# supersglzc/pql

Hardware: AMD Instinct MI355X
Metric: learner grad-steps/sec + env-steps/sec, 4096 envs batch 8192 (value = V-learner grad-steps/s at the design schedule 1 env-iteration : 4 P-steps : 8 V-steps -- critic_sample_ratio 8, critic_actor_ratio 2; weak scaling: batch-sized steps summed over ranks, strong scaling: steps of the job's batch) (higher is better)
Workload: dtype f32; 1 GPU; PQL 1xMI355X: 4096 synthetic envs (AllegroHand-shape obs=88 act=16), replay 1000000 rows resident in HBM, batch 8192, n-step 3, DoubleQ MLP [512, 512, 256]; schedule=1 env-iteration : 4 P-steps : 8 V-steps, graph=True, rng=philox, streams=True, fused_forward=True, parallelism=single, layout=single, ranks=1

## Files before the change

### pql_amd/csrc/fused.h

```cpp
#pragma once
#include "pqlk_common.h"

typedef float f32x16f __attribute__((ext_vector_type(16)));

struct FusedP {
  const float* X;
  const float* X2;
  int ldx2, x2_col0;
  const float* params;
  const float* packed;
  float* acts;
  int B, ldx, n_hidden, stash_all, buf_ld, n_nets;
  int dims[PQLK_MAX_LAYERS + 1];
  long long net_stride, packed_net_stride;
  long long b_off[PQLK_MAX_LAYERS], p_off[PQLK_MAX_LAYERS], a_off[PQLK_MAX_LAYERS];
  int head_n, head_epi, head_ld, ld_out2;
  long long head_w_off, head_b_off, head_a_off;
  const float* draw;
  float* out2;
  float* qc;
  float noise_std, noise_clip;
  const float* td_qt;
  const float* td_rew;
  const float* td_done;
// ... 16 lines not shown

template <int R, int TPW, int TM, int D, bool REFILL>
__device__ __forceinline__ void fused_group(f32x16f (&acc)[R][TPW], float4 (&bq)[D][TM], const float4* const (&wp)[TPW],
                                            const float4* __restrict__ lds4, int abase, int buf_ld4, int k8, int K8, int steps,
                                            float4 (&an)[R]) {
#pragma unroll
  for (int s = 0; s < D; ++s) {
    if (s < steps) {
      float4 a[R];
      const int kq = min(k8 + s + 1, K8 - 1);
#pragma unroll
      for (int i = 0; i < R; ++i) { a[i] = an[i]; an[i] = lds4[abase + 32 * i * buf_ld4 + 2 * kq]; }
      __builtin_amdgcn_sched_barrier(0);
      const int kn = min(k8 + s + D, K8 - 1);
#pragma unroll
      for (int t = 0; t < 4; ++t) {
#pragma unroll
        for (int j = 0; j < TPW; ++j) {
          const float bv = t == 0 ? bq[s][j].x : t == 1 ? bq[s][j].y : t == 2 ? bq[s][j].z : bq[s][j].w;
#pragma unroll
          for (int i = 0; i < R; ++i) {
            const float av = t == 0 ? a[i].x : t == 1 ? a[i].y : t == 2 ? a[i].z : a[i].w;
            acc[i][j] = __builtin_amdgcn_mfma_f32_32x32x2f32(bv, av, acc[i][j], 0, 0, 0);
          }
          if (REFILL && t == 3) {
            bq[s][j] = wp[j][kn * 64];
            __builtin_amdgcn_sched_barrier(0);
          }
        }
      }
    }
  }
}

template <int TM, int D>
__device__ __forceinline__ void fused_ring_fill(float4 (&bq)[D][TM], const float4* __restrict__ packed_l, int K8, int K8s, int ntiles, int tpw,
                                                int wave, int lane) {
  const float4* w[TM];
#pragma unroll
  for (int j = 0; j < TM; ++j) w[j] = packed_l + (long long)min(wave * tpw + j, ntiles - 1) * K8s * 64 + lane;
#pragma unroll
  for (int s = 0; s < D; ++s) {
    const int ks = min(s, K8 - 1) * 64;
#pragma unroll
    for (int j = 0; j < TM; ++j) bq[s][j] = w[j][ks];
  }
}

template <int R, int TPW, int TM, int D>
__device__ __forceinline__ void fused_layer(float4 (&bq)[D][TM], int buf_ld4, int K8, int K8s, int ntiles, const float4* __restrict__ packed_l,
                                            int bias_lds4, float* __restrict__ gout, int g_ld, int row0, int B, int wave, int lane,
                                            const float4* __restrict__ packed_n, int K8n, int ntiles_n, int tpw_n,
                                            float* __restrict__ gprev, int nprev4) {
  const int r = lane & 31, h = lane >> 5;
  const int t0 = wave * TPW;
  const bool active = t0 < ntiles;
  const float4* lds4 = reinterpret_cast<const float4*>(fsm);
  float4* gprev4 = reinterpret_cast<float4*>(gprev) + (long long)row0 * nprev4;
  const int srows = gprev ? 32 * R : 0;
  const int tid = wave * 64 + lane;
  int srow = tid / nprev4, sc4 = tid % nprev4;
  const int sdq = (64 * FUSED_NW) / nprev4, sdm = (64 * FUSED_NW) % nprev4;
  f32x16f acc[R][TPW];
#pragma unroll
  for (int i = 0; i < R; ++i)
#pragma unroll
    for (int j = 0; j < TPW; ++j)
#pragma unroll
      for (int e = 0; e < 16; ++e) acc[i][j][e] = 0.f;
  if (active) {
    const float4* wp[TPW];
#pragma unroll
    for (int j = 0; j < TPW; ++j) wp[j] = packed_l + (long long)min(t0 + j, ntiles - 1) * K8s * 64 + lane;
    const int abase = r * buf_ld4 + h;
    const int K8full = K8 - (K8 % D);
    const int G = K8full / D;
    const bool rem = K8full < K8;
    float4 an[R];
#pragma unroll
    for (int i = 0; i < R; ++i) an[i] = lds4[abase + 32 * i * buf_ld4];
    if (G > 1) fused_group<R, TPW, TM, D, true>(acc, bq, wp, lds4, abase, buf_ld4, 0, K8, D, an);
    for (int g = 1; g < G - 1; ++g) {
      if (srow < srows) {
        gprev4[(long long)srow * nprev4 + sc4] = lds4[srow * buf_ld4 + sc4];
        srow += sdq; sc4 += sdm;
        if (sc4 >= nprev4) { sc4 -= nprev4; ++srow; }
      }
      fused_group<R, TPW, TM, D, true>(acc, bq, wp, lds4, abase, buf_ld4, g * D, K8, D, an);
    }
    if (G >= 1) {
      if (rem) fused_group<R, TPW, TM, D, true>(acc, bq, wp, lds4, abase, buf_ld4, (G - 1) * D, K8, D, an);
      else fused_group<R, TPW, TM, D, false>(acc, bq, wp, lds4, abase, buf_ld4, (G - 1) * D, K8, D, an);
    }
    if (rem) fused_group<R, TPW, TM, D, false>(acc, bq, wp, lds4, abase, buf_ld4, K8full, K8, K8 - K8full, an);
  }
  while (srow < srows) {
    gprev4[(long long)srow * nprev4 + sc4] = lds4[srow * buf_ld4 + sc4];
    srow += sdq; sc4 += sdm;
    if (sc4 >= nprev4) { sc4 -= nprev4; ++srow; }
  }
  if (packed_n) fused_ring_fill<TM, D>(bq, packed_n, K8n, K8n, ntiles_n, tpw_n, wave, lane);
  __syncthreads();
  if (active) {
    float4* out4 = reinterpret_cast<float4*>(fsm);
    const bool full = row0 + 32 * R <= B;
#pragma unroll
    for (int j = 0; j < TPW; ++j) {
      if (t0 + j < ntiles) {
#pragma unroll
        for (int q = 0; q < 4; ++q) {
          const int c4 = 8 * (t0 + j) + 2 * q + h;
          const float4 b4 = lds4[bias_lds4 + c4];
#pragma unroll
          for (int i = 0; i < R; ++i) {
            const int row = row0 + 32 * i + r;
            float4 v;
            v.x = fused_elu(acc[i][j][4 * q] + b4.x);
            v.y = fused_elu(acc[i][j][4 * q + 1] + b4.y);
            v.z = fused_elu(acc[i][j][4 * q + 2] + b4.z);
            v.w = fused_elu(acc[i][j][4 * q + 3] + b4.w);
            out4[(32 * i + r) * buf_ld4 + c4] = v;
            if (gout && (full || row < B)) *reinterpret_cast<float4*>(gout + (long long)row * g_ld + 4 * c4) = v;
          }
        }
      }
    }
  }
  __syncthreads();
}

enum { HEAD_NONE = PQLK_ACT_NONE, HEAD_TANH = PQLK_ACT_TANH, HEAD_TANH_NOISE = PQLK_ACT_TANH_NOISE };

template <int R, bool TDH = true>
__device__ __forceinline__ void fused_head(const FusedP& p, const float* __restrict__ params, float* __restrict__ acts, int net, int row0,
                                           int buf_ld4, int wave, int lane) {
  constexpr int NW = FUSED_NW;
  const int r = lane & 31, h = lane >> 5;
  const int Kh = p.dims[p.n_hidden], K8 = Kh >> 3, N = p.head_n;
  const float* W = params + (long long)net * p.net_stride + p.head_w_off;
  const float4* wp = reinterpret_cast<const float4*>(W + (long long)min(r, N - 1) * Kh) + h;
  const float4* lds4 = reinterpret_cast<const float4*>(fsm);
  const int per = (K8 + NW - 1) / NW, k0 = wave * per, k1 = min(K8, k0 + per);
  f32x16f acc[R];
#pragma unroll
  for (int i = 0; i < R; ++i)
#pragma unroll
    for (int e = 0; e < 16; ++e) acc[i][e] = 0.f;
  for (int k8 = k0; k8 < k1; ++k8) {
    const float4 w4 = wp[2 * k8];
#pragma unroll
    for (int i = 0; i < R; ++i) {
      const float4 a4 = lds4[(32 * i + r) * buf_ld4 + 2 * k8 + h];
      acc[i] = __builtin_amdgcn_mfma_f32_32x32x2f32(w4.x, a4.x, acc[i], 0, 0, 0);
      acc[i] = __builtin_amdgcn_mfma_f32_32x32x2f32(w4.y, a4.y, acc[i], 0, 0, 0);
      acc[i] = __builtin_amdgcn_mfma_f32_32x32x2f32(w4.z, a4.z, acc[i], 0, 0, 0);
      acc[i] = __builtin_amdgcn_mfma_f32_32x32x2f32(w4.w, a4.w, acc[i], 0, 0, 0);
    }
  }
  const bool td = TDH && p.td_dz != nullptr;
  constexpr int TDI = 2 * R;
  float tdt[TDI], tdr[TDI], tdd[TDI];
  if (td && ((wave * 64 + lane) & 31) == 0) {
#pragma unroll
    for (int k = 0; k < TDI; ++k) {
      const long long m = min(row0 + ((wave * 64 + lane) >> 5) + 16 * k, p.B - 1);
      tdt[k] = fminf(p.td_qt[m * p.head_ld], p.td_qt[((long long)p.B + m) * p.head_ld]);
      tdr[k] = p.td_rew[m]; tdd[k] = p.td_done[m];
    }
  }
  auto part_at = [&](int x) { return td ? (x >> 8) * p.buf_ld + Kh + (x & 255) : x; };
  __syncthreads();
#pragma unroll
  for (int i = 0; i < R; ++i)
#pragma unroll
    for (int e = 0; e < 16; ++e) fsm[part_at(((wave * R + i) * 16 + e) * 64 + lane)] = acc[i][e];
  __syncthreads();
  const float* bias = params + (long long)net * p.net_stride + p.head_b_off;
  float* out = acts + p.head_a_off + (long long)net * p.B * p.head_ld;
  const int tdbase = 32 * R * p.buf_ld;
  int ok = 0;
  for (int o = wave * 64 + lane; o < 32 * R * p.head_ld; o += 64 * NW, ++ok) {
    const int row = o / p.head_ld, c = o - row * p.head_ld;
    if (row0 + row >= p.B) {
      if (td && c == 0) { fsm[tdbase + row] = 0.f; fsm[tdbase + 32 * R + row] = 0.f; }
      continue;
    }
    float x = 0.f;
    if (c < N) {
      const int i = row >> 5, ln = (row & 31) + 32 * ((c >> 2) & 1), e = 4 * (c >> 3) + (c & 3);
      float s = 0.f;
#pragma unroll
      for (int w = 0; w < NW; ++w) s += fsm[part_at(((w * R + i) * 16 + e) * 64 + ln)];
      x = s + bias[c];
      if (p.qc) p.qc[(long long)net * p.B + row0 + row] = x;
      if (td) {
        float tq = tdt[0], tr = tdr[0], tn = tdd[0];
#pragma unroll
        for (int k = 1; k < TDI; ++k)
          if (ok == k) { tq = tdt[k]; tr = tdr[k]; tn = tdd[k]; }
        const float y = tr + ((1.f - tn) * p.td_gamma_n) * tq;
        const float dq = x - y;
        fsm[tdbase + row] = p.td_two_over_b * dq;
        fsm[tdbase + 32 * R + row] = dq * dq;
      }
      if (p.head_epi == HEAD_TANH) x = tanhf(x);
      else if (p.head_epi == HEAD_TANH_NOISE) {
        x = tanhf(x);
        float nz = p.noise_std * p.draw[(long long)(row0 + row) * N + c];
        nz = fminf(fmaxf(nz, -p.noise_clip), p.noise_clip);
        x = fminf(fmaxf(x + nz, -1.f), 1.f);
      }
      if (p.out2 && net == 0) p.out2[(long long)(row0 + row) * p.ld_out2 + c] = x;
    }
    out[(long long)(row0 + row) * p.head_ld + c] = x;
  }
  if (!td) return;
  __syncthreads();
  const int kq = Kh >> 2;
  const int tile = row0 / (32 * R);
  float* dz = p.td_dz + ((long long)net * p.B + row0) * Kh;
  constexpr int RW = 32 * R / NW;
  float* hp = p.td_head_part + ((long long)tile * p.n_nets + net) * p.td_part_floats;
  for (int q0 = 0; q0 < kq; q0 += 64) {
    const int q = q0 + lane;
    float4 s = make_float4(0.f, 0.f, 0.f, 0.f);
    if (q < kq) {
      const float4 w4 = *reinterpret_cast<const float4*>(W + 4 * q);
#pragma unroll
      for (int u = 0; u < RW; ++u) {
        const int row = wave * RW + u;
        const float dn = fsm[tdbase + row];
        const float4 h4 = lds4[row * buf_ld4 + q];
        s.x += dn * h4.x; s.y += dn * h4.y; s.z += dn * h4.z; s.w += dn * h4.w;
        float4 a = make_float4(dn * w4.x, dn * w4.y, dn * w4.z, dn * w4.w);
        a.x = h4.x > 0.f ? a.x : a.x * (h4.x + 1.f);
        a.y = h4.y > 0.f ? a.y : a.y * (h4.y + 1.f);
        a.z = h4.z > 0.f ? a.z : a.z * (h4.z + 1.f);
        a.w = h4.w > 0.f ? a.w : a.w * (h4.w + 1.f);
        if (row0 + row < p.B) *reinterpret_cast<float4*>(dz + (long long)row * Kh + 4 * q) = a;
      }
    }
    __syncthreads();
    if (q < kq) *reinterpret_cast<float4*>(&fsm[wave * p.buf_ld + Kh + 4 * lane]) = s;
    __syncthreads();
    if (wave == 0 && q < kq) {
      float4 t = *reinterpret_cast<const float4*>(&fsm[Kh + 4 * lane]);
#pragma unroll
      for (int w = 1; w < NW; ++w) {
        const float4 v = *reinterpret_cast<const float4*>(&fsm[w * p.buf_ld + Kh + 4 * lane]);
        t.x += v.x; t.y += v.y; t.z += v.z; t.w += v.w;
      }
      *reinterpret_cast<float4*>(hp + 4 * q) = t;
    }
  }
  if (wave == 1) {
    float db = lane < 32 * R ? fsm[tdbase + lane] : 0.f, ls = lane < 32 * R ? fsm[tdbase + 32 * R + lane] : 0.f;
    db = wave_sum(db); ls = wave_sum(ls);
    if (lane < 32) hp[Kh + lane] = lane == 0 ? db : 0.f;
    if (lane == 0) p.td_loss_part[(long long)tile * p.n_nets + net] = ls;
  }
}

template <int R, int TM, bool OUT_ONLY = false>
__global__ __launch_bounds__(64 * FUSED_NW) void k_mlp_fwd_fused(FusedP p) {
  constexpr int NW = FUSED_NW, D = TM >= 4 ? 2 : PQLK_FUSED_DEEP;
  const int tid = threadIdx.x, lane = tid & 63, wave = tid >> 6;
  int net, tile;
  const int tiles = (p.B + 32 * R - 1) / (32 * R);
  if (p.n_nets == 2 && (tiles & 3) == 0) {
    const int b = blockIdx.x, g = b & 7, i = b >> 3;
    net = g & 1;
    tile = i * 4 + (g >> 1);
  } else {
    net = blockIdx.x / tiles;
    tile = blockIdx.x % tiles;
  }
  const float* __restrict__ pX = p.X;
  const float* __restrict__ pparams = p.params;
  const float* __restrict__ ppacked = p.packed;
  float* __restrict__ pacts = p.acts;
  const int pstash = OUT_ONLY ? 0 : p.stash_all;
  const int row0 = tile * 32 * R;
  const bool full_tile = row0 + 32 * R <= p.B;
  const int buf_ld4 = p.buf_ld >> 2;
  const float4* packed_net = reinterpret_cast<const float4*>(ppacked + (long long)net * p.packed_net_stride);
  auto tpw_of = [](int ntiles) { return ntiles > 2 * NW ? 4 : ntiles > NW ? 2 : 1; };
  float4 bq[D][TM];
  fused_ring_fill<TM, D>(bq, packed_net + (p.p_off[0] >> 2), (p.dims[0] + 7) >> 3, ((p.dims[0] + 31) & ~31) >> 3, p.dims[1] >> 5,
                         tpw_of(p.dims[1] >> 5), wave, lane);
  float4* out4 = reinterpret_cast<float4*>(fsm);
  const int bias4 = 32 * R * buf_ld4;
  {
    float4 bv[PQLK_MAX_LAYERS];
#pragma unroll
    for (int l = 0; l < PQLK_MAX_LAYERS; ++l) {
      bv[l] = make_float4(0.f, 0.f, 0.f, 0.f);
      if (l < p.n_hidden && tid < (p.dims[l + 1] >> 2))
        bv[l] = reinterpret_cast<const float4*>(pparams + (long long)net * p.net_stride + p.b_off[l])[tid];
    }
    const int k0 = (p.dims[0] + 31) & ~31, cpr = k0 >> 2, w = p.dims[0], total = 32 * R * cpr;
    for (int i0 = tid; i0 < total; i0 += 4 * 64 * NW) {
      float4 v[4];
#pragma unroll
      for (int u = 0; u < 4; ++u) {
        const int i = i0 + u * 64 * NW;
        const int row = i / cpr, c4 = i - row * cpr;
        v[u] = make_float4(0.f, 0.f, 0.f, 0.f);
        if (i < total && row0 + row < p.B) {
          const int c = 4 * c4;
          if (p.X2 && c >= p.x2_col0) {
            if (c - p.x2_col0 < p.ldx2) v[u] = *reinterpret_cast<const float4*>(p.X2 + (long long)(row0 + row) * p.ldx2 + (c - p.x2_col0));
          } else if (c < p.ldx) {
            v[u] = *reinterpret_cast<const float4*>(pX + (long long)(row0 + row) * p.ldx + c);
          }
        }
      }
#pragma unroll
      for (int u = 0; u < 4; ++u) {
        const int i = i0 + u * 64 * NW;
        if (i < total) {
          const int row = i / cpr, c4 = i - row * cpr, c = 4 * c4;
          float4 x = v[u];
// ... 65 lines not shown
```

### pql_amd/csrc/gemm.hip

```cpp
#include <cstdlib>
#include <type_traits>
#include "pqlk_common.h"
#include "skinny.h"
#include "fused.h"

typedef float f32x16 __attribute__((ext_vector_type(16)));

enum { MODE_FWD = 0, MODE_DX = 1, MODE_DW = 2 };
enum { EPI_NONE = 0, EPI_ELU = 1, EPI_TANH = 2, EPI_TANH_NOISE = 3, EPI_DELU = 4, EPI_DTANH_SLICE = 5 };

struct GemmP {
  const float* A;
  const float* B;
  float* C;
  const float* bias;
  const float* aux;
  float* C2;
  float* dbias;
  int M, N, K;
  int lda, ldb, ldc, ldaux, ldc2;
  int ncols_store;
  long long sA, sB, sC, sBias, sAux;
  int groups;
  int zsum;
// ... 362 lines not shown
        __builtin_amdgcn_sched_barrier(0);
        compute(kt, 0);
        PQLK_SS(1, 1);
        __syncthreads();
        PQLK_GL(min(kt + 3, nk - 1), 1);
        __builtin_amdgcn_sched_barrier(0);
        compute(kt + 1, 1);
        PQLK_SS(0, 0);
        __syncthreads();
      }
#undef PQLK_GL
#undef PQLK_SS
      continue;
    }

    KcTile<BM, KT> a_kc;
    RrTile<BM, KT> a_rr;
    KcTile<BN, KT> b_kc;
    RrTile<BN, KT> b_rr;

    auto gload = [&](int kt) {
      const int k0 = kbeg + kt * KT;
      if (MODE == MODE_FWD) {
        a_kc.load(A, p.lda, m0, p.M, k0, kend, tid);
        b_kc.load(B, p.ldb, n0, p.N, k0, kend, tid);
      } else if (MODE == MODE_DX) {
        a_kc.load(A, p.lda, m0, p.M, k0, p.lda, tid);
        b_rr.load(B, p.ldb, k0, kend, n0, p.ldb, tid);
      } else {
        a_rr.load(A, p.lda, k0, kend, m0, p.lda, tid);
        b_rr.load(B, p.ldb, k0, kend, n0, p.ldb, tid);
      }
    };
    auto sstore = [&](int stage) {
      float* sa = smem + stage * S::STAGE;
      float* sb = sa + S::A_FLOATS;
      if (MODE == MODE_FWD) {
        a_kc.store(sa, tid);
        b_kc.store(sb, tid);
      } else if (MODE == MODE_DX) {
        a_kc.store(sa, tid);
        b_rr.store(sb, tid);
      } else {
        a_rr.store(sa, tid);
        b_rr.store(sb, tid);
      }
    };

    gload(0);
    __syncthreads();
    sstore(0);
    __syncthreads();

    for (int kt = 0; kt < nk; ++kt) {
      const int stage = kt & 1;
      if (kt + 1 < nk) gload(kt + 1);
      compute(kt, stage);
      if (kt + 1 < nk) sstore(stage ^ 1);
      __syncthreads();
    }
  }

  if (MODE == MODE_DW && bx == 0) {
    smem[tid] = dbacc;
    __syncthreads();
    if (tid < BM) {
      dbacc = smem[tid];
#pragma unroll
      for (int g = 1; g < 256 / BM; ++g) dbacc += smem[g * BM + tid];
    }
    __syncthreads();
  }
  if (MODE != MODE_FWD && EPI != EPI_DTANH_SLICE) {
    const bool whole = (m0 + BM <= p.M) && (n0 + BN <= p.N) && (MODE == MODE_DW || !p.C2);
    if (whole) {
      constexpr int PLD = WN + 4;
      constexpr int LPR = WN / 4;
      constexpr int RPI = 64 / LPR;
      float* patch = smem + wave * (32 * PLD);
      const int gq = (MODE == MODE_DX && p.zsum) ? 0 : g0;
      float* Cw = (MODE == MODE_DW) ? p.C + (long long)g0 * p.sC + (long long)split * p.sSplit : p.C + (long long)gq * p.sC;
      const float* auxw = (EPI == EPI_DELU && p.aux) ? p.aux + (long long)gq * p.sAux : nullptr;
      const int prow = lane / LPR, pc4 = lane % LPR;
#pragma unroll
      for (int i = 0; i < MI; ++i) {
        f4v h4s[(EPI == EPI_DELU) ? 32 / RPI : 1];
        if (EPI == EPI_DELU) {
          long long arow[32 / RPI];
          const long long grow0 = m0 + wm + 32 * i + prow;
          if (MODE == MODE_DX && p.perm) {
            int pr[32 / RPI];
#pragma unroll
            for (int it = 0; it < 32 / RPI; ++it) pr[it] = p.perm[grow0 + it * RPI];
#pragma unroll
            for (int it = 0; it < 32 / RPI; ++it) arow[it] = pr[it] < 0 ? 0 : pr[it];
          } else {
#pragma unroll
            for (int it = 0; it < 32 / RPI; ++it) arow[it] = grow0 + it * RPI;
          }
#pragma unroll
          for (int it = 0; it < 32 / RPI; ++it)
            h4s[it] = *reinterpret_cast<const f4v*>(auxw + arow[it] * p.ldaux + n0 + wn + 4 * pc4);
        }
#pragma unroll
        for (int j = 0; j < NJ; ++j)
#pragma unroll
          for (int q = 0; q < 4; ++q)
            *reinterpret_cast<float4*>(patch + r * PLD + 32 * j + 8 * q + 4 * h) =
                make_float4(acc[i][j][4 * q], acc[i][j][4 * q + 1], acc[i][j][4 * q + 2], acc[i][j][4 * q + 3]);
        __builtin_amdgcn_fence(__ATOMIC_RELEASE, "wavefront");
        __builtin_amdgcn_wave_barrier();
        __builtin_amdgcn_fence(__ATOMIC_ACQUIRE, "wavefront");
#pragma unroll
        for (int it = 0; it < 32 / RPI; ++it) {
          const int rr = it * RPI + prow;
          float4 v = *reinterpret_cast<const float4*>(patch + rr * PLD + 4 * pc4);
          const long long grow = m0 + wm + 32 * i + rr;
          const int gcol = n0 + wn + 4 * pc4;
          if (EPI == EPI_DELU) {
            const f4v h4 = h4s[it];
            v.x = h4.x > 0.f ? v.x : v.x * (h4.x + 1.f);
            v.y = h4.y > 0.f ? v.y : v.y * (h4.y + 1.f);
            v.z = h4.z > 0.f ? v.z : v.z * (h4.z + 1.f);
            v.w = h4.w > 0.f ? v.w : v.w * (h4.w + 1.f);
          }
          *reinterpret_cast<float4*>(Cw + grow * p.ldc + gcol) = v;
        }
        if (i + 1 < MI) {
          __builtin_amdgcn_fence(__ATOMIC_RELEASE, "wavefront");
          __builtin_amdgcn_wave_barrier();
          __builtin_amdgcn_fence(__ATOMIC_ACQUIRE, "wavefront");
        }
      }
      if (MODE == MODE_DW && bx == 0 && tid < BM && p.dbias) {
        float* db = p.dbias + (long long)g0 * p.sBias + (long long)split * p.sSplit;
        const int row = m0 + tid;
        if (row < p.ncols_store) db[row] = row < p.M ? dbacc : 0.f;
      }
      return;
    }
  }
  if (MODE == MODE_DW) {
    float* C = p.C + (long long)g0 * p.sC + (long long)split * p.sSplit;
#pragma unroll
    for (int i = 0; i < MI; ++i)
#pragma unroll
      for (int j = 0; j < NJ; ++j) {
        const int row = m0 + wm + 32 * i + r;
#pragma unroll
        for (int q = 0; q < 4; ++q) {
          const int col = n0 + wn + 32 * j + 8 * q + 4 * h;
          if (row < p.M && col < p.N)
            *reinterpret_cast<float4*>(C + (long long)row * p.ldc + col) =
                make_float4(acc[i][j][4 * q], acc[i][j][4 * q + 1], acc[i][j][4 * q + 2], acc[i][j][4 * q + 3]);
        }
      }
    if (bx == 0 && tid < BM && p.dbias) {
      float* db = p.dbias + (long long)g0 * p.sBias + (long long)split * p.sSplit;
      const int row = m0 + tid;
      if (row < p.ncols_store) db[row] = row < p.M ? dbacc : 0.f;
    }
    return;
  }

  const int g = (MODE == MODE_DX && p.zsum) ? 0 : g0;
  float* C = p.C + (long long)g * p.sC;
  const float* bias = (MODE == MODE_FWD && p.bias) ? p.bias + (long long)g * p.sBias : nullptr;
  const float* aux = p.aux ? p.aux + (long long)g * p.sAux : nullptr;
  const bool full = (m0 + BM <= p.M) && (n0 + BN <= p.N) && EPI != EPI_DTANH_SLICE && EPI != EPI_TANH_NOISE && !p.C2;
#pragma unroll
  for (int i = 0; i < MI; ++i)
#pragma unroll
    for (int j = 0; j < NJ; ++j) {
      const int row = m0 + wm + 32 * i + r;
#pragma unroll
      for (int q = 0; q < 4; ++q) {
        const int col = n0 + wn + 32 * j + 8 * q + 4 * h;
        float v[4] = {acc[i][j][4 * q], acc[i][j][4 * q + 1], acc[i][j][4 * q + 2], acc[i][j][4 * q + 3]};
        if (full) {
          if (MODE == MODE_FWD) {
            const float4 b4 = bias ? *reinterpret_cast<const float4*>(bias + col) : make_float4(0.f, 0.f, 0.f, 0.f);
            v[0] += b4.x; v[1] += b4.y; v[2] += b4.z; v[3] += b4.w;
#pragma unroll
            for (int u = 0; u < 4; ++u) {
              if (EPI == EPI_ELU) v[u] = elu1(v[u]);
              else if (EPI == EPI_TANH) v[u] = tanhf(v[u]);
            }
          } else if (EPI == EPI_DELU) {
            const float4 h4 = *reinterpret_cast<const float4*>(aux + (long long)row * p.ldaux + col);
            v[0] = h4.x > 0.f ? v[0] : v[0] * (h4.x + 1.f);
            v[1] = h4.y > 0.f ? v[1] : v[1] * (h4.y + 1.f);
            v[2] = h4.z > 0.f ? v[2] : v[2] * (h4.z + 1.f);
            v[3] = h4.w > 0.f ? v[3] : v[3] * (h4.w + 1.f);
          }
          *reinterpret_cast<float4*>(C + (long long)row * p.ldc + col) = make_float4(v[0], v[1], v[2], v[3]);
          continue;
        }
        if (row >= p.M) continue;
#pragma unroll
        for (int u = 0; u < 4; ++u) {
          const int c = col + u;
          float x = v[u];
          if (EPI == EPI_DTANH_SLICE) {
            const int cc = c - p.col0;
            if (cc >= 0 && cc < p.ncol) {
              const float a = aux[(long long)row * p.ldaux + cc];
              C[(long long)row * p.ldc + cc] = x * (1.f - a * a);
            }
            continue;
// ... 358 lines not shown
  int rc = desc_ok(d);
  if (rc) return rc;
  PQLK_REQUIRE(params && x && acts, PQLK_E_NULL);
  PQLK_REQUIRE(b > 0 && b < (1LL << 30), PQLK_E_SHAPE);
  PQLK_REQUIRE(ldx % 32 == 0 && ldx >= pqlk_ld(d->dims[0]), PQLK_E_ALIGN);
  PQLK_REQUIRE(pqlk_aligned16(params) && pqlk_aligned16(x) && pqlk_aligned16(acts), PQLK_E_ALIGN);
  PQLK_REQUIRE(out_act == PQLK_ACT_NONE || out_act == PQLK_ACT_TANH || out_act == PQLK_ACT_TANH_NOISE, PQLK_E_UNSUPPORTED);
  if (out_act == PQLK_ACT_TANH_NOISE) PQLK_REQUIRE(draw, PQLK_E_NULL);
  if (out2) PQLK_REQUIRE(d->n_nets == 1 && ld_out2 >= d->dims[d->n_layers], PQLK_E_SHAPE);
  PQLK_REQUIRE(stash_all >= 0 && stash_all <= PQLK_STASH_OUTPUT_ONLY, PQLK_E_RANGE);
  const int64_t net_stride = pqlk_mlp_net_stride(d);
  const int L = d->n_layers;
  int l_first = 0;
  static const bool no_head = getenv("PQLK_NO_FUSED_HEAD") != nullptr;
  const bool out_only = stash_all == PQLK_STASH_OUTPUT_ONLY;
  if (out_only) PQLK_REQUIRE(packed && fusable(d, nullptr) && head_fusable(d) && !no_head, PQLK_E_UNSUPPORTED);
  if (packed && fusable(d, nullptr)) {
    PQLK_REQUIRE(pqlk_aligned16(packed), PQLK_E_ALIGN);
    FusedHead head = {};
    if (head_fusable(d) && !no_head) {
      head.n = d->dims[L]; head.epi = out_act; head.draw = draw; head.noise_std = noise_std; head.noise_clip = noise_clip;
      head.out2 = out2; head.ld_out2 = ld_out2;
    }
    rc = launch_fused_hidden(d, params, packed, x, ldx, b, acts, stash_all == 1 ? 1 : 0, pqlk_s(stream), &head, out_only);
    if (rc) return rc;
    l_first = head.n > 0 ? L : L - 1;
  }
  for (int l = l_first; l < L; ++l) {
    int64_t w_off, b_off, a_off, a_ld;
    pqlk_mlp_layer_offsets(d, l, &w_off, &b_off);
    pqlk_mlp_act_offset(d, b, 0, l, &a_off, &a_ld);
    GemmP p = {};
    if (l == 0) {
      p.A = x; p.lda = (int)ldx; p.sA = 0;
    } else {
      int64_t i_off, i_ld;
      pqlk_mlp_act_offset(d, b, 0, l - 1, &i_off, &i_ld);
      p.A = acts + i_off; p.lda = (int)i_ld; p.sA = b * i_ld;
    }
    p.B = params + w_off; p.ldb = (int)pqlk_ld(d->dims[l]); p.sB = net_stride;
    p.bias = params + b_off; p.sBias = net_stride;
    p.C = acts + a_off; p.ldc = (int)a_ld; p.sC = b * a_ld;
    p.M = (int)b; p.N = d->dims[l + 1]; p.K = (int)pqlk_ld(d->dims[l]);
    p.ncols_store = (int)a_ld;
    p.groups = d->n_nets;
    p.epi = EPI_ELU;
    if (l == L - 1) {
      p.epi = out_act == PQLK_ACT_TANH ? EPI_TANH : (out_act == PQLK_ACT_TANH_NOISE ? EPI_TANH_NOISE : EPI_NONE);
      p.aux = draw; p.sAux = 0;
      p.noise_std = noise_std; p.noise_clip = noise_clip;
      p.C2 = out2; p.ldc2 = (int)ld_out2;
    }
    if (l == L - 1 && skinny_fwd_ok(d->dims[l + 1], p.K)) {
      SkinnyP q = {};
      q.X = p.A; q.ldx = p.lda; q.sX = p.sA;
      q.W = p.B; q.ldk = p.ldb; q.sW = p.sB;
      q.bias = p.bias; q.sBias = p.sBias;
      q.C = p.C; q.ldc = p.ldc; q.sC = p.sC;
      q.M = p.M; q.N = p.N; q.K = p.K;
      q.epi = p.epi == EPI_TANH ? SK_EPI_TANH : (p.epi == EPI_TANH_NOISE ? SK_EPI_TANH_NOISE : SK_EPI_NONE);
      q.draw = p.aux; q.noise_std = noise_std; q.noise_clip = noise_clip;
      q.C2 = p.C2; q.ldc2 = p.ldc2;
      rc = launch_skinny_fwd(q, d->n_nets, pqlk_s(stream));
    } else if (l == L - 1 && narrow_fwd_ok(p)) {
      rc = launch_fwd_narrow(p, d->n_nets, pqlk_s(stream));
    } else {
      rc = launch_auto<MODE_FWD>(p, d->n_nets, pqlk_s(stream));
    }
    if (rc) return rc;
  }
  return PQLK_OK;
}

struct ReduceP {
  const float* slabs; int splits; long long n;
  float* out;
  const float* head_part; int head_parts; int n_nets; long long net_stride, head_off, head_floats;
  long long seg_off, seg_len;
  int main_blocks;
  float* sq_part; int32_t* step_dev;
  const int* parts_dev;
};

__global__ __launch_bounds__(256) void k_reduce_slabs(ReduceP p) {
  __shared__ float shw[4];
  float acc = 0.f;
  if ((int)blockIdx.x < p.main_blocks) {
    const long long sq = p.seg_len >> 2, n4 = sq * p.n_nets;
    for (long long i = (long long)blockIdx.x * 256 + threadIdx.x; i < n4; i += (long long)p.main_blocks * 256) {
      long long q = i, base = p.seg_off;
      while (q >= sq) { q -= sq; base += p.net_stride; }
      if (p.head_parts > 0 && p.seg_off + (q << 2) >= p.head_off) continue;
      const long long off = base + (q << 2);
      float4 s = *reinterpret_cast<const float4*>(p.slabs + off);
      for (int k = 1; k < p.splits; ++k) {
        const float4 t = *reinterpret_cast<const float4*>(p.slabs + (long long)k * p.n + off);
        s.x += t.x; s.y += t.y; s.z += t.z; s.w += t.w;
      }
      *reinterpret_cast<float4*>(p.out + off) = s;
      acc += (s.x * s.x + s.y * s.y) + (s.z * s.z + s.w * s.w);
    }
    if (!p.sq_part) return;
    acc = wave_sum(acc);
  } else {
    const int lane = threadIdx.x & 63;
    const long long hq = p.head_floats >> 2;
    const long long e = ((long long)blockIdx.x - p.main_blocks) * 4 + (threadIdx.x >> 6);
    if (e < hq * p.n_nets) {
      const long long net = e / hq, q = e - net * hq;
      const float* hp = p.head_part + net * p.head_floats + 4 * q;
      float4 s = make_float4(0.f, 0.f, 0.f, 0.f);
      const int parts = p.parts_dev ? min(p.head_parts, (p.parts_dev[3] + 31) / 32) : p.head_parts;
      for (int k = lane; k < parts; k += 64) {
        const float4 t = *reinterpret_cast<const float4*>(hp + (long long)k * p.n_nets * p.head_floats);
        s.x += t.x; s.y += t.y; s.z += t.z; s.w += t.w;
      }
      s.x = wave_sum(s.x); s.y = wave_sum(s.y); s.z = wave_sum(s.z); s.w = wave_sum(s.w);
      if (lane == 0) *reinterpret_cast<float4*>(p.out + net * p.net_stride + p.head_off + 4 * q) = s;
      acc = (s.x * s.x + s.y * s.y) + (s.z * s.z + s.w * s.w);
    }
    if (!p.sq_part) return;
  }
  if ((threadIdx.x & 63) == 0) shw[threadIdx.x >> 6] = acc;
  __syncthreads();
  if (threadIdx.x == 0) {
    p.sq_part[blockIdx.x] = (shw[0] + shw[1]) + (shw[2] + shw[3]);
    if (blockIdx.x == 0 && p.step_dev) p.step_dev[0] += 1;
  }
}

static int64_t head_quads(const PqlMlpDesc* d) {
  const int L = d->n_layers;
  return ((int64_t)d->dims[L] * pqlk_ld(d->dims[L - 1]) + pqlk_ld(d->dims[L])) / 4 * d->n_nets;
}
static bool head_is_fused(const PqlMlpDesc* d) {
  const int L = d->n_layers;
  return L >= 2 && skinny_bwd_ok(d->dims[L], (int)pqlk_ld(d->dims[L - 1])) && skinny_bwd_fused_ok(d->dims[L], (int)pqlk_ld(d->dims[L - 1]));
}
static int reduce_main_blocks(int64_t arena, bool for_norm) {
  int64_t blocks = (arena / 4 + 255) / 256;
  if (blocks < 1) blocks = 1;
  const int64_t cap = for_norm ? 1024 : 2048;
  return (int)(blocks > cap ? cap : blocks);
}

extern "C" int32_t pqlk_mlp_norm_parts(const PqlMlpDesc* d) {
  if (desc_ok(d)) return 0;
  const int main_blocks = reduce_main_blocks(pqlk_mlp_param_floats(d), true);
  return main_blocks + (head_is_fused(d) ? (int)((head_quads(d) + 3) / 4) : 0);
}

struct TdHead {
  const float* qt; const float* rew; const float* done; float gamma_n; float* loss_part;
};

static int mlp_backward_impl(const PqlMlpDesc* d, const float* params, const float* x, int64_t ldx, int64_t b,
                             const float* acts, const float* dy, float* grads, int32_t splits, float* dx,
                             int64_t ld_dx, int32_t dx_col0, int32_t dx_cols, const float* dx_tanh_of,
                             int64_t ld_tanh, float* ws, int64_t ws_floats, float* sq_part, int32_t* step_dev,
                             pqlk_stream_t stream, const TdHead* td = nullptr, int l_hi = -1, int l_lo = 0, int head_done = 0,
                             const int* head_parts_dev = nullptr) {
  int rc = desc_ok(d);
  if (rc) return rc;
  const bool ranged = l_hi >= 0;
  if (!ranged) l_hi = d->n_layers - 1;
  PQLK_REQUIRE(l_lo >= 0 && l_lo <= l_hi && l_hi < d->n_layers, PQLK_E_RANGE);
  PQLK_REQUIRE(!ranged || (grads && !dx && !sq_part), PQLK_E_UNSUPPORTED);
  PQLK_REQUIRE(params && x && acts && (dy || td || head_done || l_hi < d->n_layers - 1) && ws, PQLK_E_NULL);
  PQLK_REQUIRE(!head_done || (!ranged && grads && !dx && !td && d->n_layers >= 2), PQLK_E_UNSUPPORTED);
  if (td) PQLK_REQUIRE(grads && d->n_nets == 2 && d->dims[d->n_layers] == 1 && head_is_fused(d), PQLK_E_UNSUPPORTED);
  PQLK_REQUIRE(b > 0 && b < (1LL << 30), PQLK_E_SHAPE);
  PQLK_REQUIRE(ldx % 32 == 0 && ldx >= pqlk_ld(d->dims[0]), PQLK_E_ALIGN);
  PQLK_REQUIRE(grads || dx, PQLK_E_NULL);
  if (grads) PQLK_REQUIRE(splits >= 1 && splits <= 64, PQLK_E_SHAPE);
  if (!grads) splits = 0;
  PQLK_REQUIRE(ws_floats >= 2 * (int64_t)d->n_nets * b * max_hidden_ld(d) + (int64_t)splits * pqlk_mlp_param_floats(d) +
                                (grads ? head_part_floats(d, b) : 0), PQLK_E_WORKSPACE);
  PQLK_REQUIRE(!sq_part || grads, PQLK_E_NULL);
  if (dx) {
    PQLK_REQUIRE(ld_dx % 32 == 0, PQLK_E_ALIGN);
// ... 43 lines not shown
          pqlk_mlp_act_offset(d, b, 0, L - 1, &q_off, &q_ld);
          PQLK_REQUIRE(in_ld >= ld_in && q_ld == ld_out, PQLK_E_SHAPE);
          q.td_q = acts + q_off; q.td_qt = td->qt; q.td_rew = td->rew; q.td_done = td->done;
          q.td_gamma_n = td->gamma_n; q.td_two_over_b = 2.0f / (float)b; q.td_part = td->loss_part;
        }
        rc = launch_skinny_bwd(q, d->n_nets, head_part, (long long)(net_stride - w_off), st);
        if (rc) return rc;
        continue;
      }
      if (grads) {
        q.dW = slabs + w_off; q.dB = slabs + b_off; q.sW = net_stride; q.sBias = net_stride; q.sSplit = arena;
        q.splits = splits; q.rows_per_split = (int)pqlk_round_up((b + splits - 1) / splits, KT_MAX);
        rc = launch_skinny_dw(q, d->n_nets, st);
        if (rc) return rc;
      }
      if (l > 0) {
        q.W = params + w_off; q.sW = net_stride;
        q.C = dact[flip]; q.sC = b * ld_in;
        q.epi = SK_EPI_DELU;
        rc = launch_skinny_dx(q, d->n_nets, st);
        if (rc) return rc;
        continue;
      }
      if (!dx) continue;
    }
    if (grads && !skinny) {
      GemmP p = {};
      p.A = cur_dy; p.lda = (int)ld_out; p.sA = b * ld_out;
      p.B = in; p.ldb = (int)in_ld; p.sB = in_stride;
      p.C = slabs + w_off; p.ldc = (int)ld_in; p.sC = net_stride;
      p.dbias = slabs + b_off; p.sBias = net_stride;
      p.M = d->dims[l + 1]; p.N = (int)ld_in; p.K = (int)b;
      p.ncols_store = (int)ld_out;
      p.groups = d->n_nets; p.splits = splits;
      p.rows_per_split = (int)pqlk_round_up((b + splits - 1) / splits, KT_MAX);
      p.sSplit = arena;
      rc = launch_auto<MODE_DW>(p, d->n_nets * splits, st);
      if (rc) return rc;
    }
    if (l > 0) {
      GemmP p = {};
      p.A = cur_dy; p.lda = (int)ld_out; p.sA = b * ld_out;
      p.B = params + w_off; p.ldb = (int)ld_in; p.sB = net_stride;
      p.C = dact[flip]; p.ldc = (int)ld_in; p.sC = b * ld_in;
      p.aux = in; p.ldaux = (int)in_ld; p.sAux = in_stride;
      p.M = (int)b; p.N = d->dims[l]; p.K = d->dims[l + 1];
      p.ncols_store = (int)ld_in;
      p.groups = d->n_nets; p.zsum = 0;
      p.epi = EPI_DELU;
      rc = launch_auto<MODE_DX>(p, d->n_nets, st);
      if (rc) return rc;
    } else if (dx) {
      GemmP p = {};
      p.A = cur_dy; p.lda = (int)ld_out; p.sA = b * ld_out;
      p.B = params + w_off; p.ldb = (int)ld_in; p.sB = net_stride;
      p.C = dx; p.ldc = (int)ld_dx; p.sC = 0;
      p.M = (int)b; p.N = d->dims[0]; p.K = d->dims[1];
      p.ncols_store = (int)ld_in;
      p.groups = d->n_nets; p.zsum = 1;
      if (dx_tanh_of) {
        p.epi = EPI_DTANH_SLICE; p.aux = dx_tanh_of; p.ldaux = (int)ld_tanh; p.col0 = dx_col0; p.ncol = dx_cols;
      } else {
        p.epi = EPI_NONE;
      }
      if (dx_slice_ok(p)) rc = launch_dx_slice(p, st);
      else rc = launch_auto<MODE_DX>(p, 1, st);
      if (rc) return rc;
    }
  }
  if (grads) {
    ReduceP r = {};
    r.slabs = slabs; r.splits = splits; r.n = arena; r.out = grads;
    r.head_part = head_part; r.head_parts = head_blocks; r.n_nets = d->n_nets; r.net_stride = net_stride;
    int64_t w_last, b_last, w_lo, w_next, b_tmp;
    pqlk_mlp_layer_offsets(d, L - 1, &w_last, &b_last);
    r.head_off = w_last; r.head_floats = net_stride - w_last;
    pqlk_mlp_layer_offsets(d, l_lo, &w_lo, &b_tmp);
    w_next = net_stride;
    if (l_hi < L - 1) pqlk_mlp_layer_offsets(d, l_hi + 1, &w_next, &b_tmp);
    r.seg_off = w_lo; r.seg_len = w_next - w_lo;
    r.sq_part = sq_part; r.step_dev = step_dev; r.parts_dev = head_parts_dev;
    r.main_blocks = reduce_main_blocks(r.seg_len * d->n_nets, sq_part != nullptr);
    const int extra = head_blocks > 0 ? (int)((head_quads(d) + 3) / 4) : 0;
    hipLaunchKernelGGL(k_reduce_slabs, dim3(r.main_blocks + extra), dim3(256), 0, st, r);
    PQLK_LAUNCH_CHECK();
  }
  return PQLK_OK;
}

static bool minnet_ok(const PqlMlpDesc* d, const float* dx, const float* dx_tanh_of, int dx_cols) {
  const int L = d->n_layers;
  if (d->n_nets != 2 || L < 3 || d->dims[L] != 1 || !dx || !dx_tanh_of || dx_cols > 32) return false;
  if (!skinny_bwd_ok(1, (int)pqlk_ld(d->dims[L - 1]))) return false;
  for (int l = 1; l < L; ++l)
    if (d->dims[l] % 32 != 0) return false;
  for (int l = 1; l < L - 1; ++l)
    if (d->dims[l] % 128 != 0) return false;
  return true;
}
static int64_t minnet_rows_cap(int64_t b) { return 2 * pqlk_round_up(b, MN_TILE); }

static int launch_compact_dx(const GemmP& p, bool first, hipStream_t st) {
  static const int ctile = [] { const char* e = getenv("PQLK_COMPACT_TILE"); return e ? atoi(e) : 2; }();
  const bool small = ctile == 2 || (ctile == 3 && first) || (ctile == 4 && !first);
  if (ctile == 1) return launch_gemm<MODE_DX, 128, 128, EPI_DELU>(p, 1, st);
  if (small) return launch_gemm<MODE_DX, 64, 64, EPI_DELU>(p, 1, st);
  return launch_gemm<MODE_DX, 128, 64, EPI_DELU>(p, 1, st);
}

extern "C" int64_t pqlk_dpg_backward_ws_floats(const PqlMlpDesc* d, int64_t b) {
  if (desc_ok(d) || b <= 0) return 0;
  const int64_t dense = pqlk_mlp_bwd_ws_floats(d, b, 1);
  const int64_t compact = 2 * minnet_rows_cap(b) * max_hidden_ld(d) + 2 * minnet_rows_cap(b) + 64;
  return dense > compact ? dense : compact;
}

extern "C" int pqlk_dpg_critic_backward(const PqlMlpDesc* d, const float* params, const float* x, int64_t ldx, int64_t b,
                                        const float* acts, const float* dy, float* dx, int64_t ld_dx, int32_t dx_col0,
                                        int32_t dx_cols, const float* dx_tanh_of, int64_t ld_tanh, const uint8_t* owner, float* ws,
                                        int64_t ws_floats, pqlk_stream_t stream) {
  int rc = desc_ok(d);
  if (rc) return rc;
  PQLK_REQUIRE(ws_floats >= pqlk_dpg_backward_ws_floats(d, b), PQLK_E_WORKSPACE);
  if (!minnet_ok(d, dx, dx_tanh_of, dx_cols) || b > 131072)
    return mlp_backward_impl(d, params, x, ldx, b, acts, dy, nullptr, 1, dx, ld_dx, dx_col0, dx_cols, dx_tanh_of, ld_tanh, ws, ws_floats,
                             nullptr, nullptr, stream);
  PQLK_REQUIRE(params && acts && dy && ws, PQLK_E_NULL);
  PQLK_REQUIRE(b > 0 && b < (1LL << 29), PQLK_E_SHAPE);
  PQLK_REQUIRE(ld_dx % 32 == 0 && dx_col0 >= 0 && dx_cols > 0 && dx_col0 + dx_cols <= d->dims[0] && ld_dx >= dx_cols, PQLK_E_RANGE);
  const int L = d->n_layers;
  const int64_t net_stride = pqlk_mlp_net_stride(d);
  const int64_t rows_cap = minnet_rows_cap(b), mld = max_hidden_ld(d);
  float* dz[2] = {ws, ws + rows_cap * mld};
  int* perm = reinterpret_cast<int*>(ws + 2 * rows_cap * mld);
  int* mn = perm + rows_cap;
  hipStream_t st = pqlk_s(stream);
  int64_t q_off, q_ld;
  pqlk_mlp_act_offset(d, b, 0, L - 1, &q_off, &q_ld);
  hipLaunchKernelGGL(k_minnet_partition, dim3(1), dim3(1024), 0, st, owner, acts + q_off, q_ld, b, perm, rows_cap, mn);
  PQLK_LAUNCH_CHECK();
  {
    int64_t w_off, b_off, h_off, h_ld;
    pqlk_mlp_layer_offsets(d, L - 1, &w_off, &b_off);
    pqlk_mlp_act_offset(d, b, 0, L - 2, &h_off, &h_ld);
    MinnetHeadP h = {};
    h.H = acts + h_off; h.sH = b * h_ld; h.ldh = (int)h_ld;
    h.W = params + w_off; h.sW = net_stride; h.ldk = (int)pqlk_ld(d->dims[L - 1]);
    h.dY = dy; h.sY = b * pqlk_ld(1); h.ldy = (int)pqlk_ld(1);
    h.C = dz[0]; h.perm = perm; h.mn = mn; h.N = 1; h.K = h.ldk; h.rows_cap = rows_cap;
    h.zero_out = dx; h.zero_floats = b * ld_dx;
    int64_t blocks = rows_cap / 4;
    if (blocks > 2048) blocks = 2048;
    hipLaunchKernelGGL(k_minnet_head_dx, dim3((unsigned)blocks), dim3(256), (size_t)2 * h.N * h.K * sizeof(float), st, h);
    PQLK_LAUNCH_CHECK();
  }
  int flip = 0;
  for (int l = L - 2; l >= 1; --l) {
    int64_t w_off, b_off, a_off, a_ld;
    pqlk_mlp_layer_offsets(d, l, &w_off, &b_off);
    pqlk_mlp_act_offset(d, b, 0, l - 1, &a_off, &a_ld);
    GemmP p = {};
    p.A = dz[flip]; p.lda = (int)pqlk_ld(d->dims[l + 1]); p.sA = 0;
    p.B = params + w_off; p.ldb = (int)pqlk_ld(d->dims[l]); p.sB = net_stride;
    p.C = dz[flip ^ 1]; p.ldc = (int)pqlk_ld(d->dims[l]); p.sC = 0;
    p.aux = acts + a_off; p.ldaux = (int)a_ld; p.sAux = b * a_ld;
    p.M = (int)rows_cap; p.N = d->dims[l]; p.K = d->dims[l + 1];
    p.ncols_store = p.ldc;
// ... 294 lines not shown
```

### pql_amd/csrc/pqlk_common.h

```cpp
#pragma once
#include <hip/hip_runtime.h>
#include <stdint.h>

#include <atomic>
#include <mutex>

#include "../../include/pqlk.h"

#define PQLK_WAVE 64

#define PQLK_REQUIRE(cond, code) \
  do {                           \
    if (!(cond)) return (code);  \
  } while (0)

#define PQLK_LAUNCH_CHECK()                    \
  do {                                         \
    hipError_t e__ = hipGetLastError();        \
    if (e__ != hipSuccess) return -(int)e__;   \
  } while (0)

static inline int64_t pqlk_round_up(int64_t x, int64_t m) { return (x + m - 1) / m * m; }
static inline hipStream_t pqlk_s(pqlk_stream_t s) { return (hipStream_t)s; }
static inline bool pqlk_aligned16(const void* p) { return (((uintptr_t)p) & 15u) == 0; }

struct RecLayout {
  int O, A;
  int o4, a4;
  int off_nobs, off_act, off_rd;
  int used;
  int ld;
};

__host__ __device__ static inline RecLayout rec_layout(int O, int A) {
  RecLayout L;
  L.O = O; L.A = A;
  L.o4 = (O + 3) & ~3;
  if (A < 0) {
    L.a4 = 0; L.off_nobs = L.off_act = L.off_rd = L.o4; L.used = L.o4;
  } else {
    L.a4 = (A + 3) & ~3;
    L.off_nobs = L.o4; L.off_act = 2 * L.o4; L.off_rd = 2 * L.o4 + L.a4; L.used = L.off_rd + 4;
  }
  L.ld = (L.used + 31) & ~31;
  return L;
}

struct RecLayoutH {
  int O, A;
  int oh;
  int off_nobs, off_act, off_rd;
  int used;
  int ld;
};

__host__ __device__ static inline RecLayoutH rec_layout_h(int O, int A) {
  RecLayoutH L;
  L.O = O; L.A = A;
  L.oh = ((O + 7) & ~7) >> 1;
  if (A < 0) {
    L.off_nobs = L.off_act = L.off_rd = L.oh; L.used = L.oh;
  } else {
    L.off_nobs = L.oh; L.off_act = 2 * L.oh; L.off_rd = 2 * L.oh + ((A + 3) & ~3); L.used = L.off_rd + 4;
  }
  L.ld = (L.used + 31) & ~31;
  return L;
}

struct PqlkPerDeviceOnce {
  std::atomic<bool> done[64] = {};
  std::mutex mu;
  template <class F>
  int run(F&& f) {
    int dev = 0;
    if (hipGetDevice(&dev) != hipSuccess || dev < 0 || dev >= 64) return f();
    if (done[dev].load(std::memory_order_acquire)) return 0;
    std::lock_guard<std::mutex> g(mu);
    if (done[dev].load(std::memory_order_relaxed)) return 0;
    const int rc = f();
    if (rc == 0) done[dev].store(true, std::memory_order_release);
    return rc;
  }
};

__device__ __forceinline__ float wave_sum(float v) {
#pragma unroll
  for (int o = 32; o > 0; o >>= 1) v += __shfl_xor(v, o, 64);
  return v;
}
__device__ __forceinline__ float wave_max(float v) {
#pragma unroll
  for (int o = 32; o > 0; o >>= 1) v = fmaxf(v, __shfl_xor(v, o, 64));
  return v;
}
```

Baseline: 1218 V-learner grad-steps/s.

## Use write-through buffer stores for activations and templated split reduction

Adds a helper that issues raw buffer b128 stores with a cache-policy bit, and uses it for activation stash, dz, and backward GEMM epilogue stores. Full-tile activation writes to global memory move to a coalesced pass from LDS after the barrier. The slab reduction kernel gets compile-time split counts (8 and 16) so loads can be unrolled and issued together. The intent is to cut cache pollution and store overhead and to raise memory-level parallelism in the reduction. The cost is 32-bit offset limits in the buffer resource (int indices) and an extra LDS read pass.

```diff
diff --git a/pql_amd/csrc/fused.h b/pql_amd/csrc/fused.h
--- a/pql_amd/csrc/fused.h
+++ b/pql_amd/csrc/fused.h
@@ -122,7 +122,7 @@
     if (G > 1) fused_group<R, TPW, TM, D, true>(acc, bq, wp, lds4, abase, buf_ld4, 0, K8, D, an);
     for (int g = 1; g < G - 1; ++g) {
       if (srow < srows) {
-        gprev4[(long long)srow * nprev4 + sc4] = lds4[srow * buf_ld4 + sc4];
+        pqlk_store_wt(gprev4, srow * nprev4 + sc4, lds4[srow * buf_ld4 + sc4]);
         srow += sdq; sc4 += sdm;
         if (sc4 >= nprev4) { sc4 -= nprev4; ++srow; }
       }
@@ -135,7 +135,7 @@
     if (rem) fused_group<R, TPW, TM, D, false>(acc, bq, wp, lds4, abase, buf_ld4, K8full, K8, K8 - K8full, an);
   }
   while (srow < srows) {
-    gprev4[(long long)srow * nprev4 + sc4] = lds4[srow * buf_ld4 + sc4];
+    pqlk_store_wt(gprev4, srow * nprev4 + sc4, lds4[srow * buf_ld4 + sc4]);
     srow += sdq; sc4 += sdm;
     if (sc4 >= nprev4) { sc4 -= nprev4; ++srow; }
   }
@@ -160,13 +160,21 @@
             v.z = fused_elu(acc[i][j][4 * q + 2] + b4.z);
             v.w = fused_elu(acc[i][j][4 * q + 3] + b4.w);
             out4[(32 * i + r) * buf_ld4 + c4] = v;
-            if (gout && (full || row < B)) *reinterpret_cast<float4*>(gout + (long long)row * g_ld + 4 * c4) = v;
+            if (gout && !full && row < B) *reinterpret_cast<float4*>(gout + (long long)row * g_ld + 4 * c4) = v;
           }
         }
       }
     }
   }
   __syncthreads();
+  if (gout && row0 + 32 * R <= B) {
+    float4* g4 = reinterpret_cast<float4*>(gout + (long long)row0 * g_ld);
+    const int n4 = g_ld >> 2, total = 32 * R * n4;
+    for (int e = tid; e < total; e += 64 * FUSED_NW) {
+      const int row = e / n4;
+      pqlk_store_wt(g4, e, lds4[row * buf_ld4 + (e - row * n4)]);
+    }
+  }
 }
 
 enum { HEAD_NONE = PQLK_ACT_NONE, HEAD_TANH = PQLK_ACT_TANH, HEAD_TANH_NOISE = PQLK_ACT_TANH_NOISE };
@@ -277,7 +285,7 @@
         a.y = h4.y > 0.f ? a.y : a.y * (h4.y + 1.f);
         a.z = h4.z > 0.f ? a.z : a.z * (h4.z + 1.f);
         a.w = h4.w > 0.f ? a.w : a.w * (h4.w + 1.f);
-        if (row0 + row < p.B) *reinterpret_cast<float4*>(dz + (long long)row * Kh + 4 * q) = a;
+        if (row0 + row < p.B) pqlk_store_wt(reinterpret_cast<float4*>(dz), row * kq + q, a);
       }
     }
     __syncthreads();
diff --git a/pql_amd/csrc/gemm.hip b/pql_amd/csrc/gemm.hip
--- a/pql_amd/csrc/gemm.hip
+++ b/pql_amd/csrc/gemm.hip
@@ -468,6 +468,7 @@
       float* Cw = (MODE == MODE_DW) ? p.C + (long long)g0 * p.sC + (long long)split * p.sSplit : p.C + (long long)gq * p.sC;
       const float* auxw = (EPI == EPI_DELU && p.aux) ? p.aux + (long long)gq * p.sAux : nullptr;
       const int prow = lane / LPR, pc4 = lane % LPR;
+      float4* Cb = reinterpret_cast<float4*>(Cw + (long long)m0 * p.ldc + n0);
 #pragma unroll
       for (int i = 0; i < MI; ++i) {
         f4v h4s[(EPI == EPI_DELU) ? 32 / RPI : 1];
@@ -501,8 +502,6 @@
         for (int it = 0; it < 32 / RPI; ++it) {
           const int rr = it * RPI + prow;
           float4 v = *reinterpret_cast<const float4*>(patch + rr * PLD + 4 * pc4);
-          const long long grow = m0 + wm + 32 * i + rr;
-          const int gcol = n0 + wn + 4 * pc4;
           if (EPI == EPI_DELU) {
             const f4v h4 = h4s[it];
             v.x = h4.x > 0.f ? v.x : v.x * (h4.x + 1.f);
@@ -510,7 +509,7 @@
             v.z = h4.z > 0.f ? v.z : v.z * (h4.z + 1.f);
             v.w = h4.w > 0.f ? v.w : v.w * (h4.w + 1.f);
           }
-          *reinterpret_cast<float4*>(Cw + grow * p.ldc + gcol) = v;
+          pqlk_store_wt(Cb, ((wm + 32 * i + rr) * p.ldc + wn + 4 * pc4) >> 2, v);
         }
         if (i + 1 < MI) {
           __builtin_amdgcn_fence(__ATOMIC_RELEASE, "wavefront");
@@ -1035,6 +1034,7 @@
   const int* parts_dev;
 };
 
+template <int SPLITS>
 __global__ __launch_bounds__(256) void k_reduce_slabs(ReduceP p) {
   __shared__ float shw[4];
   float acc = 0.f;
@@ -1045,10 +1045,20 @@
       while (q >= sq) { q -= sq; base += p.net_stride; }
       if (p.head_parts > 0 && p.seg_off + (q << 2) >= p.head_off) continue;
       const long long off = base + (q << 2);
-      float4 s = *reinterpret_cast<const float4*>(p.slabs + off);
-      for (int k = 1; k < p.splits; ++k) {
-        const float4 t = *reinterpret_cast<const float4*>(p.slabs + (long long)k * p.n + off);
-        s.x += t.x; s.y += t.y; s.z += t.z; s.w += t.w;
+      float4 s;
+      if constexpr (SPLITS > 0) {
+        float4 t[SPLITS];
+#pragma unroll
+        for (int k = 0; k < SPLITS; ++k) t[k] = *reinterpret_cast<const float4*>(p.slabs + (long long)k * p.n + off);
+        s = t[0];
+#pragma unroll
+        for (int k = 1; k < SPLITS; ++k) { s.x += t[k].x; s.y += t[k].y; s.z += t[k].z; s.w += t[k].w; }
+      } else {
+        s = *reinterpret_cast<const float4*>(p.slabs + off);
+        for (int k = 1; k < p.splits; ++k) {
+          const float4 t = *reinterpret_cast<const float4*>(p.slabs + (long long)k * p.n + off);
+          s.x += t.x; s.y += t.y; s.z += t.z; s.w += t.w;
+        }
       }
       *reinterpret_cast<float4*>(p.out + off) = s;
       acc += (s.x * s.x + s.y * s.y) + (s.z * s.z + s.w * s.w);
@@ -1258,7 +1268,10 @@
     r.sq_part = sq_part; r.step_dev = step_dev; r.parts_dev = head_parts_dev;
     r.main_blocks = reduce_main_blocks(r.seg_len * d->n_nets, sq_part != nullptr);
     const int extra = head_blocks > 0 ? (int)((head_quads(d) + 3) / 4) : 0;
-    hipLaunchKernelGGL(k_reduce_slabs, dim3(r.main_blocks + extra), dim3(256), 0, st, r);
+    const dim3 rgrid(r.main_blocks + extra);
+    if (splits == 16) hipLaunchKernelGGL(k_reduce_slabs<16>, rgrid, dim3(256), 0, st, r);
+    else if (splits == 8) hipLaunchKernelGGL(k_reduce_slabs<8>, rgrid, dim3(256), 0, st, r);
+    else hipLaunchKernelGGL(k_reduce_slabs<0>, rgrid, dim3(256), 0, st, r);
     PQLK_LAUNCH_CHECK();
   }
   return PQLK_OK;
diff --git a/pql_amd/csrc/pqlk_common.h b/pql_amd/csrc/pqlk_common.h
--- a/pql_amd/csrc/pqlk_common.h
+++ b/pql_amd/csrc/pqlk_common.h
@@ -93,3 +93,10 @@
   for (int o = 32; o > 0; o >>= 1) v = fmaxf(v, __shfl_xor(v, o, 64));
   return v;
 }
+
+__device__ __forceinline__ void pqlk_store_wt(float4* base, int idx, const float4& v) {
+  typedef unsigned pqlk_u4v __attribute__((ext_vector_type(4)));
+  const __amdgpu_buffer_rsrc_t rsrc = __builtin_amdgcn_make_buffer_rsrc(base, 0, 0x7fffffff, 0x00020000);
+  __builtin_amdgcn_raw_buffer_store_b128(pqlk_u4v{__float_as_uint(v.x), __float_as_uint(v.y), __float_as_uint(v.z), __float_as_uint(v.w)}, rsrc,
+                                         idx * 16, 0, 16 );
+}
```

New measurement: 1226 V-learner grad-steps/s (median of 6 runs). Within noise of the previous version (+0.6%).
